# bharath-raghavan/enflow

Measured on AMD Instinct MI355X. Metric: molecule-transforms/sec (fwd+log|detJ|), batch 1024×22 atoms, 1/2/4/8 GPU, higher is better.
Workload: dtype f32 (f16x3 GEMMs); 1 GPU; lf_forward_1024x22_L8_H128_nf5_f32; molecules_per_gpu=1024, atoms_per_molecule=22, coupling_layers=8, hidden_nf=128, node_nf=5, global_batch=1024, parallelism=single GPU

## Files before the change

enflow_amd/_lib.py:

```python
import ctypes
import os

import torch

_HERE = os.path.dirname(os.path.abspath(__file__))
LIB_PATH = os.environ.get("ENFLOW_LIB") or os.path.join(_HERE, "libenflow_hip.so")
LIB_NF16_PATH = os.environ.get("ENFLOW_LIB_NF16") or os.path.join(_HERE, "libenflow_hip_nf16.so")
BASE_NFMAX = 8
MAX_NODE_NF = 16
TRAIN_MAX_NODE_NF = 16

ERR_TOO_MANY_ATOMS = 1
ERR_FEW_IMAGES = 2
ERR_TOO_MANY_FEATURES = 4
ERR_RANGE = 8
ERR_SMALL = 16
ERR_HANDOFF = 32
ERR_RERUN = ERR_RANGE | ERR_SMALL
DEQUANT_NONE, DEQUANT_ARGMAX, DEQUANT_FLOOR = 0, 1, 2
PREC_F32, PREC_F16X3, PREC_BF16 = 0, 1, 2
PRECISIONS = {"f32": PREC_F32, "f16x3": PREC_F16X3, "bf16": PREC_BF16}
PREC_NO_SPLIT = 0x400
EGCL_ATTENTION, EGCL_NORM_DIFF, EGCL_TANH, EGCL_ACT = 1, 2, 4, 8
EGCL_VARIANTS = 0x100
BWD_F32 = 0x200

_i, _i64, _f, _p = ctypes.c_int, ctypes.c_int64, ctypes.c_float, ctypes.c_void_p
_u64 = ctypes.c_uint64

SIGNATURES = {
    "enflow_abi_version": (_i, []),
    "enflow_set_latency_threshold": (_i, [_i]),
    "enflow_latency_threshold": (_i, []),
    "enflow_set_split_threshold": (_i, [_i]),
    "enflow_set_fs_threshold": (_i, [_i]),
    "enflow_set_handoff_spin_limit": (_i, [_i]),
    "enflow_set_dequant_ahead": (_i, [_i]),
    "enflow_set_longest_first": (_i, [_i]),
    "enflow_longest_first_order_f32": (_i, [_i, _i, _p, _p, _p, _p, _i, _i, _p, _p, _p]),
    "enflow_max_atoms": (_i, []),
    "enflow_max_node_nf": (_i, []),
    "enflow_supports_hidden": (_i, [_i]),
    "enflow_egcl_packed_size": (_i64, [_i, _i]),
    "enflow_argmax_packed_size": (_i64, [_i, _i]),
    "enflow_pack_egcl_f32": (_i, [_p, _i, _i, _p, _p]),
    "enflow_pack_egcl_ex_f32": (_i, [_p, _i, _i, _i, _p, _p, _p]),
    "enflow_pack_egcl_act_f32": (_i, [_p, _i, _i, _i, _i, _f, _f, _p, _p, _p]),
    "enflow_pack_argmax_f32": (_i, [_p, _i, _i, _p, _p]),
    "enflow_lf_forward_f32": (_i, [_i, _i, _i, _i, _i, _p, _p, _p, _p, _p, _p, _p, _p, _i,
                                   _i, _p, _p, _f, _f, _f, _p, _p, _p, _p, _p, _p, _i, _p]),
    "enflow_lf_reverse_f32": (_i, [_i, _i, _i, _i, _i, _p, _p, _p, _p, _p, _p, _p, _p, _i,
                                   _i, _f, _f, _p, _p, _p, _i, _p]),
    "enflow_lf_forward_io_f32": (_i, [_i, _i, _i, _i, _i, _p, _p, _p, _p, _p, _p, _p, _p, _p, _p, _p, _p, _i,
                                      _i, _p, _p, _u64, _u64, _f, _f, _f, _p, _p, _p, _p, _p, _p, _p, _i, _p]),
    "enflow_lf_reverse_io_f32": (_i, [_i, _i, _i, _i, _i, _p, _p, _p, _p, _p, _p, _p, _p, _p, _p, _p, _p, _i,
                                      _i, _f, _f, _p, _p, _p, _i, _p]),
    "enflow_lf_forward_io2_f32": (_i, [_i, _i, _i, _i, _i, _p, _p, _p, _p, _p, _p, _p, _p, _p, _p, _p, _p, _i,
                                       _i, _p, _p, _u64, _u64, _f, _f, _f, _p, _p, _p, _p, _p, _p, _p, _i,
                                       _p, _p, _i, _p]),
    "enflow_lf_reverse_io2_f32": (_i, [_i, _i, _i, _i, _i, _p, _p, _p, _p, _p, _p, _p, _p, _p, _p, _p, _p, _i,
                                       _i, _f, _f, _p, _p, _p, _i, _p, _p, _i, _p]),
    "enflow_lf_large_workspace_size": (_i64, [_i, _i, _i, _i]),
    "enflow_lf_forward_large_f32": (_i, [_i, _i, _i, _i, _i, _p, _p, _p, _p, _p, _p, _p, _p, _i,
                                         _i, _p, _p, _f, _f, _f, _p, _p, _p, _i, _p, _p, _p, _i64, _p]),
    "enflow_lf_reverse_large_f32": (_i, [_i, _i, _i, _i, _i, _p, _p, _p, _p, _p, _p, _p, _p, _i,
                                         _i, _f, _f, _p, _p, _p, _i, _p, _i64, _p]),
    "enflow_egcl_forward_large_f32": (_i, [_i, _i, _i, _i, _i, _p, _p, _p, _p, _p, _p, _f,
                                           _p, _p, _p, _p, _i, _p, _i64, _p]),
    "enflow_neighbour_pairs_large_f32": (_i, [_i, _i, _i, _p, _p, _p, _p, _p, _p, _p, _p, _i64, _p]),
    "enflow_edge_list_workspace_size": (_i64, [_i, _i]),
    "enflow_edge_list_count_f32": (_i, [_i, _i, _p, _p, _p, _p, _p, _p, _p, _i64, _p]),
# ... 55 lines not shown
        return LIB_PATH
    if int(nf) <= MAX_NODE_NF:
        return LIB_NF16_PATH
    raise NotImplementedError(f"enflow_amd kernels are built for node_nf <= {MAX_NODE_NF} (got {nf})")


def lib(nf=None):
    path = lib_path(nf)
    handle = _libs.get(path)
    if handle is None:
        if not os.path.exists(path):
            raise HipPathError(
                f"{path} is missing: build it with "
                "`python -c 'import __graft_entry__ as g; g.build()'` (hipcc --offload-arch=gfx950)")
        handle = ctypes.CDLL(path)
        for name, (res, args) in SIGNATURES.items():
            if not hasattr(handle, name):
                continue
            fn = getattr(handle, name)
            fn.restype = res
            fn.argtypes = args
        if _lat_threshold[0] is not None and hasattr(handle, "enflow_set_latency_threshold"):
            handle.enflow_set_latency_threshold(_lat_threshold[0])
        if _split_threshold[0] is not None and hasattr(handle, "enflow_set_split_threshold"):
            handle.enflow_set_split_threshold(_split_threshold[0])
        if _fs_threshold[0] is not None and hasattr(handle, "enflow_set_fs_threshold"):
            handle.enflow_set_fs_threshold(_fs_threshold[0])
        if _spin_limit[0] is not None and hasattr(handle, "enflow_set_handoff_spin_limit"):
            handle.enflow_set_handoff_spin_limit(_spin_limit[0])
        if _dq_ahead[0] is not None and hasattr(handle, "enflow_set_dequant_ahead"):
            handle.enflow_set_dequant_ahead(_dq_ahead[0])
        if _longest_first[0] is not None and hasattr(handle, "enflow_set_longest_first"):
            handle.enflow_set_longest_first(_longest_first[0])
        _libs[path] = handle
    return handle


_lat_threshold = [None]


def set_latency_threshold(max_mols):
    prev = _lat_threshold[0]
    _lat_threshold[0] = int(max_mols)
    for h in _libs.values():
        if hasattr(h, "enflow_set_latency_threshold"):
            h.enflow_set_latency_threshold(int(max_mols))
    return prev


_split_threshold = [None]
_fs_threshold = [None]
_spin_limit = [None]
_dq_ahead = [None]


def set_dequant_ahead(on):
    prev = _dq_ahead[0]
    _dq_ahead[0] = 1 if on else 0
    for h in _libs.values():
        if hasattr(h, "enflow_set_dequant_ahead"):
            h.enflow_set_dequant_ahead(_dq_ahead[0])
    return prev


_longest_first = [None]


def set_longest_first(mode):
    prev = _longest_first[0]
    _longest_first[0] = int(mode)
    for h in _libs.values():
        if hasattr(h, "enflow_set_longest_first"):
            h.enflow_set_longest_first(int(mode))
    return prev


def longest_first_order(mol_ptr, r_cut, box, pos, max_mol_atoms, reverse=False, training=False):
    num_mols = int(mol_ptr.numel()) - 1
    keys = torch.full((max(num_mols, 1),), -1, dtype=torch.int32, device=pos.device)
    order = torch.full((max(num_mols, 1),), -1, dtype=torch.int32, device=pos.device)
    rc = lib().enflow_longest_first_order_f32(num_mols, int(max_mol_atoms), ptr(mol_ptr), ptr(r_cut), ptr(box),
                                              ptr(pos), int(bool(reverse)), int(bool(training)), ptr(keys),
                                              ptr(order), stream_ptr(pos.device))
    if rc < 0:
        raise HipPathError(f"enflow_longest_first_order_f32 failed with code {rc}")
    return keys[:num_mols], order[:num_mols], bool(rc)


def set_handoff_spin_limit(polls):
    prev = _spin_limit[0]
    _spin_limit[0] = int(polls)
    for h in _libs.values():
        if hasattr(h, "enflow_set_handoff_spin_limit"):
            h.enflow_set_handoff_spin_limit(int(polls))
    return prev


def set_split_threshold(max_mols):
    prev = _split_threshold[0]
    _split_threshold[0] = int(max_mols)
    for h in _libs.values():
        if hasattr(h, "enflow_set_split_threshold"):
            h.enflow_set_split_threshold(int(max_mols))
    return prev


# ... 186 lines not shown
```

enflow_amd/csrc/enflow_flow.hip:

```cpp

#include <mutex>
#include "enflow_large.h"
#include "enflow_host.h"
#include "enflow_latency.h"
#include "enflow_split.h"

__device__ __forceinline__ void pack_egcl_body(const float* __restrict__ raw, int H, int nf, float* __restrict__ out,
                                               int flags, const float* __restrict__ att, int act_kind, float act_p0,
                                               float act_p1) {
  const EgclLayout L = egcl_layout(H, nf);
  const RawEgcl R = raw_egcl(H, nf);
  const int NT = H / 32;
  const int K1 = 2 * nf + 1;
  for (int idx = blockIdx.x * blockDim.x + threadIdx.x; idx < L.total; idx += gridDim.x * blockDim.x) {
    float v = 0.f;
    if (idx < L.we2f) {
      int e = idx - L.we1f;
      int lane = e & 63, slot = (e >> 6) % (NFMAX + 1), t = (e >> 6) / (NFMAX + 1);
      int hh = lane >> 5;
      int q = -1;
      if (slot < NFMAX / 2) { int f = 2 * slot + hh; if (f < nf) q = f; }
      else if (slot < NFMAX) { int f = 2 * (slot - NFMAX / 2) + hh; if (f < nf) q = nf + f; }
      else if (hh == 0) q = 2 * nf;
      if (q >= 0) v = raw[R.We1 + (32 * t + (lane & 31)) * K1 + q];
// ... 544 lines not shown
    *b = DqBuf{dev, st, 0, 0, nullptr, nullptr};
  }
  if (b->cap_z < nz) {
    float* p = nullptr;
    const size_t c = nz < 65536 ? 65536 : nz;
    if (hipMalloc(&p, c * sizeof(float)) != hipSuccess) return nullptr;
    b->z = p;
    b->cap_z = c;
  }
  if (b->cap_m < nm) {
    float* p = nullptr;
    const size_t c = nm < 4096 ? 4096 : nm;
    if (hipMalloc(&p, c * sizeof(float)) != hipSuccess) return nullptr;
    b->lq = p;
    b->cap_m = c;
  }
  return b;
}
static int g_cus[64];
static int cus_now() {
  int dev = 0;
  if (hipGetDevice(&dev) != hipSuccess) return 0;
  if (dev < 0 || dev >= 64) return 0;
  if (g_cus[dev] == 0) {
    int cus = 0;
    if (hipDeviceGetAttribute(&cus, hipDeviceAttributeMultiprocessorCount, dev) != hipSuccess || cus <= 0) return 0;
    g_cus[dev] = cus;
  }
  return g_cus[dev];
}
static int lat_threshold_now() { return g_lat_threshold >= 0 ? g_lat_threshold : cus_now(); }

static int g_longest_first = LONGEST_FIRST_DEFAULT;
struct OrdBuf {
  int dev;
  hipStream_t st;
  size_t cap;
  int32_t* key;
};
static OrdBuf g_ord[64];
static int g_nord = 0;
static int32_t* order_buffers(hipStream_t st, size_t nm) {
  int dev = 0;
  if (hipGetDevice(&dev) != hipSuccess) return nullptr;
  std::lock_guard<std::mutex> lk(g_dq_mu);
  OrdBuf* b = nullptr;
  for (int i = 0; i < g_nord; ++i)
    if (g_ord[i].dev == dev && g_ord[i].st == st) b = &g_ord[i];
  if (!b) {
    if (g_nord >= 64) return nullptr;
    b = &g_ord[g_nord++];
    *b = OrdBuf{dev, st, 0, nullptr};
  }
  if (b->cap < nm) {
    int32_t* p = nullptr;
    const size_t c = nm < 4096 ? 4096 : nm;
    if (hipMalloc(&p, 2 * c * sizeof(int32_t)) != hipSuccess) return nullptr;
    b->key = p;
    b->cap = c;
  }
  return b->key;
}
static bool longest_first_applies(int NN, int grid, bool rev, bool tape) {
  if (g_longest_first == 0 || NN > 64 || grid < 1 || grid > ORDER_MAX_MOLS) return false;
  if (g_longest_first >= 2) return true;
  (void)rev;
  return NN == 32 && !tape && grid > 2 * cus_now();
}
template <int NN>
static void launch_order(int num_mols, hipStream_t st, const FlowArgs& A, int32_t* keys, int32_t* order) {
  ENFLOW_TIMED("order_key_kernel", st,
               hipLaunchKernelGGL((order_key_kernel<NN>), dim3(num_mols), dim3(BLOCK), 0, st, A, keys));
  ENFLOW_TIMED("order_rank_kernel", st,
               hipLaunchKernelGGL(order_rank_kernel, dim3((num_mols + 63) / 64), dim3(BLOCK), 0, st, keys, num_mols,
                                  order));
}

template <int HH, int NN, int RBB, bool REV>
static void launch_flow(int prec, int num_mols, hipStream_t st, const FlowArgs& A0) {
  if (NN == 32 && !(prec & ENFLOW_PREC_NO_SPLIT) && enflow_fs_launch(HH, REV, prec, num_mols, st, &A0)) return;
  prec &= ~ENFLOW_PREC_NO_SPLIT;
  FlowArgs A = A0;
  if constexpr (RBB == NN && NN <= 64) {
    if (A.mol_list == nullptr && longest_first_applies(NN, num_mols, REV, A.tape != nullptr)) {
      int32_t* const buf = order_buffers(st, (size_t)A.num_mols);
      if (buf != nullptr && A.num_mols == num_mols) {
        launch_order<NN>(num_mols, st, A, buf, buf + num_mols);
        A.order = buf + num_mols;
      }
    }
  }
  if (NN == 32 && num_mols <= lat_threshold_now() && enflow_lat_launch(HH, REV, prec, num_mols, st, &A)) return;
  if (prec & ENFLOW_EGCL_VARIANTS) launch_flow_v<HH, NN, RBB, REV, true>(prec & 0xff, num_mols, st, A);
  else launch_flow_v<HH, NN, RBB, REV, false>(prec, num_mols, st, A);
}

extern "C" {

#ifdef ENFLOW_STAMPS
int enflow_read_stamps(unsigned long long* host_out, int reset) {
  if (hipMemcpyFromSymbol(host_out, HIP_SYMBOL(enflow_stamp_acc), sizeof(unsigned long long) * NSTAMP) != hipSuccess)
    return -2;
  if (reset) {
    unsigned long long z[NSTAMP] = {0};
    if (hipMemcpyToSymbol(HIP_SYMBOL(enflow_stamp_acc), z, sizeof(z)) != hipSuccess) return -2;
  }
  return NSTAMP;
}
#endif

#ifdef ENFLOW_STAMPS
int enflow_read_dq_stamps(unsigned long long* host_out, int reset) {
  if (hipMemcpyFromSymbol(host_out, HIP_SYMBOL(enflow_dq_stamp_acc), sizeof(unsigned long long) * 8) != hipSuccess)
    return -2;
  if (reset) {
    unsigned long long z[8] = {0};
    if (hipMemcpyToSymbol(HIP_SYMBOL(enflow_dq_stamp_acc), z, sizeof(z)) != hipSuccess) return -2;
  }
  return 8;
}
#endif

int enflow_abi_version(void) { return ENFLOW_ABI; }
int enflow_set_dequant_ahead(int on) {
  const int prev = g_dq_ahead;
  g_dq_ahead = on ? 1 : 0;
  return prev;
}
int enflow_set_longest_first(int mode) {
  const int prev = g_longest_first;
  g_longest_first = mode < 0 ? 0 : (mode > 2 ? 2 : mode);
  return prev;
}
int enflow_longest_first_order_f32(int num_mols, int max_mol_atoms, const int32_t* mol_ptr, const float* r_cut,
                                   const float* box, const float* pos, int reverse, int training,
                                   int32_t* keys, int32_t* order, void* stream) {
  if (num_mols < 0 || max_mol_atoms < 0 || (num_mols > 0 && (!mol_ptr || !r_cut || !box || !pos || !keys || !order)))
    return -1;
  if (max_mol_atoms > 64 || num_mols > ORDER_MAX_MOLS) return 0;
  const int NN = max_mol_atoms <= 32 ? 32 : 64;
  const int applies = longest_first_applies(NN, num_mols, reverse != 0, training != 0) ? 1 : 0;
  if (num_mols == 0) return applies;
  FlowArgs A{mol_ptr, r_cut, box, nullptr, nullptr, const_cast<float*>(pos), nullptr, nullptr, 0, 1,
             0, nullptr, nullptr, 0.f, 0.f, 0.f, nullptr, nullptr, nullptr, nullptr, nullptr};
  A.num_mols = num_mols;
  if (NN == 32) launch_order<32>(num_mols, S(stream), A, keys, order);
  else launch_order<64>(num_mols, S(stream), A, keys, order);
  return hipGetLastError() == hipSuccess ? applies : -2;
}
int enflow_set_latency_threshold(int max_mols) {
  const int prev = g_lat_threshold;
  g_lat_threshold = max_mols < 0 ? -1 : max_mols;
  return prev;
}
int enflow_latency_threshold(void) { return lat_threshold_now(); }
int enflow_max_atoms(void) { return MAX_ATOMS; }
int enflow_max_node_nf(void) { return NFMAX; }
int enflow_supports_hidden(int hidden_nf) { return hid_ok(hidden_nf); }

int64_t enflow_egcl_packed_size(int hidden_nf, int node_nf) {
  if (!hid_ok(hidden_nf) || node_nf < 1 || node_nf > NFMAX) return -1;
  return egcl_layout(hidden_nf, node_nf).total;
}
int64_t enflow_argmax_packed_size(int hidden_nf, int node_nf) {
// ... 306 lines not shown
```

enflow_amd/csrc/flow_device.h:

```cpp
#pragma once

#include <hip/hip_runtime.h>
#include <stdint.h>
#include <math.h>
#include <type_traits>

#include "enflow_hip.h"
#include "enflow_timing.h"

#define ENFLOW_ABI 13
#ifndef WAVES
#define WAVES 4
#endif
#define BLOCK (64 * WAVES)
#ifndef ENFLOW_NFMAX
#define ENFLOW_NFMAX 8
#endif
#define NFMAX ENFLOW_NFMAX
static_assert(NFMAX == 8 || NFMAX == 16, "ENFLOW_NFMAX must be 8 or 16");
#define KS0MAX (NFMAX / 8 + 1)
#ifndef ENFLOW_MSG_MFMA
#define ENFLOW_MSG_MFMA 1
#endif
#define NFP (NFMAX + 1)
#ifndef ENFLOW_WAVES_PER_SIMD
#define ENFLOW_WAVES_PER_SIMD 2
#endif

typedef float f32x16 __attribute__((ext_vector_type(16)));
typedef float f32x4 __attribute__((ext_vector_type(4)));

__host__ __device__ constexpr int rho(int r, int hh) { return (r & 3) + 8 * (r >> 2) + 4 * hh; }

__host__ __device__ inline int node_ksteps(int H, int nf) { return (H + nf + 1) / 2; }

struct EgclLayout {
  int we1f, we2f, wc1f, wn1h, wn1a, wv1f, wn2f, be1, be2, bc1, wc2, bn1, bv1, wv2, bn2, bv2, watt, batt, vfl,
      scl, we1x, wv1x, wn1hx, wn1ax, wn2x, we2x, wc1x, we2b, wc1b, total;
};

enum { EGCL_ATTENTION = 1, EGCL_NORM_DIFF = 2, EGCL_TANH = 4 };

enum { PREC_F32 = 0, PREC_F16X3 = 1, PREC_BF16 = 2 };

__host__ __device__ inline EgclLayout egcl_layout(int H, int nf) {
  (void)nf;
  const int NT = H / 32;
  EgclLayout L;
  int o = 0;
  L.we1f = o; o += NT * (NFMAX + 1) * 64;
  L.we2f = o; o += H * H;
  L.wc1f = o; o += H * H;
  L.wn1h = o; o += NT * (NFMAX / 2) * 64;
  L.wn1a = o; o += NT * (H / 8) * 256;
  L.wv1f = o; o += NT * (NFMAX / 2) * 64;
// ... 796 lines not shown
#pragma unroll
    for (int g4 = 0; g4 < 4; ++g4) {
      const f32x4 v = ld4(b + 32 * t + 8 * g4 + 4 * hh);
#pragma unroll
      for (int u = 0; u < 4; ++u) acc[t][4 * g4 + u] = v[u];
    }
}

template <int NT>
__device__ __forceinline__ void bias_silu(f32x16 (&X)[NT], const float* __restrict__ bias, int hh) {
#pragma unroll
  for (int t = 0; t < NT; ++t)
#pragma unroll
    for (int g4 = 0; g4 < 4; ++g4) {
      const f32x4 b = *reinterpret_cast<const f32x4*>(bias + 32 * t + 8 * g4 + 4 * hh);
#pragma unroll
      for (int u = 0; u < 4; ++u) X[t][4 * g4 + u] = silu_f(X[t][4 * g4 + u] + b[u]);
      __builtin_amdgcn_sched_barrier(0);
    }
}

#if defined(ENFLOW_STAMPS) || (defined(ENFLOW_STAMPS_BWD) && defined(ENFLOW_BACKWARD_TU))
#define NSTAMP 20
__device__ unsigned long long enflow_stamp_acc[NSTAMP];
#define STAMP_DECL unsigned long long st_prev = __builtin_amdgcn_s_memtime(), st_acc[NSTAMP] = {0};
#define STAMP_ARGS , unsigned long long& st_prev, unsigned long long (&st_acc)[NSTAMP]
#define STAMP_PASS , st_prev, st_acc
#define STAMP(k)                                               \
  do {                                                         \
    unsigned long long now_ = __builtin_amdgcn_s_memtime();    \
    st_acc[k] += now_ - st_prev;                               \
    st_prev = now_;                                            \
  } while (0)
#define STAMP_FLUSH                                                              \
  if (threadIdx.x == 0)                                                          \
    for (int k_ = 0; k_ < NSTAMP; ++k_) atomicAdd(&enflow_stamp_acc[k_], st_acc[k_]);
#else
#define STAMP_DECL
#define STAMP_ARGS
#define STAMP_PASS
#define STAMP(k) do {} while (0)
#define STAMP_FLUSH
#endif

template <int H, int NMAX, int RB = NMAX, bool BWD = false>
struct Smem {
  static constexpr int NT = H / 32;
  static constexpr int AST = BWD ? H + 3 : H + 4;
  static constexpr bool BLOCKED = RB < NMAX;
  static constexpr bool PACKC = BLOCKED || BWD;
  static constexpr int MAXP = RB * (NMAX - 1);
  static constexpr int PC = BLOCKED ? 512 : MAXP;
  static constexpr int CW = PACKC ? (RB * NMAX + 1) / 2 : RB * NMAX;
  static constexpr int NETA = BWD ? 1 : (BLOCKED ? RB : NMAX);
  static constexpr int NBCH = 8;
  static constexpr int NBW = BWD ? (NBCH * 2 * H > WAVES * NMAX * (NFMAX + 3) ? NBCH * 2 * H
                                                                             : WAVES * NMAX * (NFMAX + 3))
                                 : 1;
  float pos[NMAX * 3], vel[NMAX * 3], boxa[BLOCKED ? 3 : NMAX * 3];
  float h[NMAX * NFP], g[NMAX * NFP], G[BWD ? 1 : NMAX * NFP];
  float Q[NMAX];
  float F[BLOCKED ? NMAX * 3 : 1];
  alignas(16) float bias[4 * H];
  static constexpr bool W1X_LDS = !BLOCKED && !BWD && NMAX <= 32;
  alignas(16) float w1x[W1X_LDS ? NT * KS0MAX * 512 : 4];
  alignas(16) float agg[RB * AST];
  alignas(16) float head[BWD ? 1 : WAVES][BWD ? 1 : H + 4];
  uint32_t pairs[PC];
  uint32_t mask27[NMAX];
  static constexpr bool IMG_LDS = W1X_LDS && NT * KS0MAX * 512 >= NMAX * 27 * 4;
  uint32_t near27[IMG_LDS ? NMAX : 1];
  float bbox[8];
  int idmap[NMAX];
  int cntrow[NMAX];
  int headrow[WAVES];
  int ishead[WAVES];
  int scan[WAVES];
  int npairs;
  int ptotal;
  int err;
  uint32_t big;
  float red[WAVES];
  static constexpr int NDT = BWD ? 1 : NT, NDR = BWD ? 1 : RB;
  static constexpr bool MSG_MMA = ENFLOW_MSG_MFMA && !BWD && NMAX == 32 && RB == 32;
  static constexpr int MIS = 34;
  union {
    int C[CW];
    struct {
      alignas(16) uint32_t img[MSG_MMA ? WAVES : 1][MSG_MMA ? 32 * MIS : 1];
      alignas(16) uint32_t tb[MSG_MMA ? WAVES : 1][32];
      int rt[MSG_MMA ? WAVES : 1][32];
    } mm;
    struct { float qp[NDT][NDR]; float gp[NDT][NFMAX][NDR]; } nd;
    float net[NETA * 2 * NFMAX];
    float nb[NBW];
  } u;
};

template <class S>
__device__ __forceinline__ int c_get(const S& sm, int e) {
  if constexpr (S::PACKC) return (sm.u.C[e >> 1] >> (16 * (e & 1))) & 0xffff;
  else return sm.u.C[e];
}
template <class S>
__device__ __forceinline__ void c_add(S& sm, int e, int v) {
  if constexpr (S::PACKC) atomicAdd(&sm.u.C[e >> 1], v << (16 * (e & 1)));
  else atomicAdd(&sm.u.C[e], v);
}

struct MolRef {
  int a0, n;
  float rc;
  float bx, by, bz;
  int m = 0;
};

__device__ __forceinline__ float shift_of(int idx, float b) { return idx == 0 ? -b : (idx == 1 ? b : 0.f); }

template <class S>
__device__ __forceinline__ void build_images(S& sm, const MolRef& M, int tid) {
  const int n = M.n;
  const float rx = M.bx + M.rc, ry = M.by + M.rc, rz = M.bz + M.rc;
  for (int a = tid; a < n; a += BLOCK) {
    sm.mask27[a] = 0u;
// ... 164 lines not shown
    }
  }
  if (tid == BLOCK - 1) {
    int tot = 0;
    for (int k = 0; k < WAVES; ++k) tot += sm.scan[k];
    sm.ptotal = tot;
    sm.npairs = min(tot - p0, PC);
  }
  __syncthreads();
  return sm.ptotal;
}

template <class S>
__device__ __forceinline__ void build_block_pairs(S& sm, const MolRef& M, int tid, int r0, int rb) {
  static_assert(!S::BLOCKED, "blocked images compact in passes (block_compact)");
  block_counts(sm, M, tid, r0, rb, r0 == 0 && rb == M.n);
  block_compact(sm, M.n, tid, rb, 0);
}

template <class S>
__device__ __forceinline__ void build_pairs(S& sm, const MolRef& M, int tid) {
  static_assert(!S::BLOCKED, "build_pairs needs the unblocked image");
  build_images(sm, M, tid);
  build_block_pairs(sm, M, tid, 0, M.n);
}

template <bool BIG>
__device__ __forceinline__ int pair_row(uint32_t pr) { return BIG ? (int)(pr & 31u) : (int)(pr & 0xffu); }

template <int H, int NMAX, int RB, int PREC = PREC_F32, bool VAR = false, bool BIG = false, class Pre = NoMid>
__device__ __forceinline__ void edge_tiles(Smem<H, NMAX, RB>& sm, const float* __restrict__ Lp, const EgclLayout& L,
                                           const MolRef& M, int nf, int tid, int r0, int rb,
                                           bool zero_agg STAMP_ARGS, const float* __restrict__ cpos = nullptr,
                                           const float* __restrict__ ch = nullptr, Pre&& pre = NoMid{}) {
  constexpr int NT = H / 32;
  constexpr int AST = Smem<H, NMAX, RB>::AST;
  const int lane = tid & 63, w = __builtin_amdgcn_readfirstlane(tid >> 6);
  const int j = lane & 31, hh = lane >> 5;
  const int P = sm.npairs;
  const int T = (P + 31) >> 5;
  const int tpw = (T + WAVES - 1) / WAVES;

  if (zero_agg)
    for (int e = tid; e < rb * AST; e += BLOCK) sm.agg[e] = 0.f;
  for (int e = tid; e < WAVES * (H + 4); e += BLOCK) (&sm.head[0][0])[e] = 0.f;
  const float K0 = PREC != PREC_F32 ? Lp[L.scl + 4] : 1.f;
  const float K1 = PREC == PREC_F16X3 ? Lp[L.scl + 0] : 1.f;
  const float K2 = PREC == PREC_F16X3 ? Lp[L.scl + 2] : 1.f;
  for (int k = tid; k < H; k += BLOCK) {
    sm.bias[k] = Lp[L.be1 + k] * K0;
    sm.bias[H + k] = Lp[L.be2 + k] * K1;
    sm.bias[2 * H + k] = Lp[L.bc1 + k] * K2;
    sm.bias[3 * H + k] = Lp[L.wc2 + k];
  }
  if constexpr (PREC != PREC_F32 && Smem<H, NMAX, RB>::W1X_LDS) {
    const int ks_n = gemm0_ksteps(nf);
    for (int e = tid; e < NT * ks_n * 128; e += BLOCK) {
      const int blk = e >> 7, r = e & 127, ln = r >> 1, part = r & 1;
      const int t = blk / ks_n, ks = blk - t * ks_n;
      const f32x4 v = ld4(Lp + L.we1x + (t * KS0MAX + ks) * 512 + ln * 8 + part * 4);
      st4(&sm.w1x[(t * KS0MAX + ks) * 512 + part * 256 + ln * 4], v);
    }
  }
  if (tid < WAVES) {
    const int t0 = tid * tpw;
    int hr = -1, ih = 0;
    if (t0 < T) {
      const int p0 = t0 * 32;
      hr = pair_row<BIG>(sm.pairs[p0]);
      ih = (p0 > 0) && (pair_row<BIG>(sm.pairs[p0 - 1]) == hr);
    }
    sm.headrow[tid] = hr;
    sm.ishead[tid] = ih;
  }
  __syncthreads();

  const int t0 = w * tpw, t1 = min(T, t0 + tpw);
  const int headrow = sm.headrow[w];
  const bool ishead = sm.ishead[w] != 0;
  const int nh = (nf + 1) >> 1;
  const rsrc_t W = weights_rsrc(Lp, L.total);
  const float hbx = M.bx * 0.5f, hby = M.by * 0.5f, hbz = M.bz * 0.5f;
  constexpr float NLOG2E = -1.4426950408889634f;
  const float ik0 = PREC != PREC_F32 ? Lp[L.scl + 5] : 1.f;
  const float ik1 = PREC == PREC_F16X3 ? Lp[L.scl + 1] : 1.f;
  const float ik2 = PREC == PREC_F16X3 ? Lp[L.scl + 3] : 1.f;
  const float c0 = NLOG2E * ik0, c1 = NLOG2E * ik1, c2 = NLOG2E * ik2;
  constexpr bool MMA = PREC != PREC_F32 && !VAR && !BIG && Smem<H, NMAX, RB>::MSG_MMA;
  constexpr int XD = (NMAX == 32 && RB == 32 && WAVES == 4 && !BIG) ? ENFLOW_FWD_X3_DEPTH : ENFLOW_X3_DEPTH;
  constexpr int MIS = Smem<H, NMAX, RB>::MIS;
  const int vfl = VAR ? (int)Lp[L.vfl] : 0;
  const bool v_att = (vfl & EGCL_ATTENTION) != 0, v_nd = (vfl & EGCL_NORM_DIFF) != 0,
             v_tanh = (vfl & EGCL_TANH) != 0;
  const Act act = VAR ? act_of(Lp + L.vfl + 1) : act_silu();

  bool range_bad = false;
  constexpr bool GUARD = PREC == PREC_F16X3;
  uint32_t bigw = 0u;
  STAMP(8);
  for (int tile = t0; tile < t1; ++tile) {
    const int p = tile * 32 + j;
    const bool valid = p < P;
    uint32_t o0 = 0u, o1 = 0u, o2 = 0u;
    const uint32_t vmask = valid ? ENFLOW_BIG_BITS : 0u;
    auto seen_big = [&](uint32_t o, uint32_t kind) {
      if constexpr (GUARD) bigw |= __ballot((o & vmask) != 0u) ? kind : 0u;
    };
    const uint32_t pr = valid ? sm.pairs[p] : 0u;
    const int il = pair_row<BIG>(pr);
    const int jl = BIG ? (int)((pr >> 5) & 0x3fffffu) : (int)((pr >> 8) & 0xffu);
// ... 288 lines not shown
                                             e[t + 1][4 * g4 + 3]}, c1, K1, ik1, act);
#pragma unroll
          for (int u = 0; u < 4; ++u) e[t + 1][4 * g4 + u] = y[u];
        }
      }, NoMid{}, [&](int, const f16x8& bh, const f16x8&) {
        if constexpr (GUARD) o2 = or_hi(o2, bh);
      });
      seen_big(o2, BIGK_M);
#pragma unroll
      for (int tp = 0; tp < NT; ++tp)
#pragma unroll
        for (int g4 = 0; g4 < 4; ++g4) {
          const f32x4 w2 = *reinterpret_cast<const f32x4*>(sm.bias + 3 * H + 32 * tp + 8 * g4 + 4 * hh);
          const f32x4 y = act4s<VAR>((f32x4){hc[tp][4 * g4], hc[tp][4 * g4 + 1], hc[tp][4 * g4 + 2],
                                             hc[tp][4 * g4 + 3]}, c2, K2, ik2, act);
#pragma unroll
          for (int u = 0; u < 4; ++u) part += w2[u] * y[u];
        }
    }
    float phi = part + __shfl_xor(part, 32, 64);
    if constexpr (PREC != PREC_F32) range_bad |= valid && !__builtin_isfinite(phi);
    if (v_tanh) phi = tanhf(phi);
    const float nd = v_nd ? __builtin_amdgcn_rcpf(sqrtf(radial) + 1.f) : 1.f;
    f32x4* const fslot = reinterpret_cast<f32x4*>(dst_row + H);
    const f32x4 fold = *fslot;
    float tx = c * clamp100(dx * nd * phi);
    float ty = c * clamp100(dy * nd * phi);
    float tz = c * clamp100(dz * nd * phi);
    float tw = 0.f;
    seg_scan4x(tx, ty, tz, tw, SE);
    if (seg_end && hh == 0) *fslot = fold + (f32x4){tx, ty, tz, tw};
    STAMP(14);
  }
  if constexpr (PREC != PREC_F32) {
    if (__ballot(range_bad))
      if (lane == 0) atomicOr(&sm.err, ENFLOW_ERR_RANGE);
  }
  if constexpr (GUARD) {
    if (lane == 0 && t1 > t0) atomicOr(&sm.big, bigw | (uint32_t)BIGK_EDGE);
  }
  pre();
  __syncthreads();
  STAMP(15);
  for (int f = tid; f < H + 3; f += BLOCK) {
    for (int ww = 0; ww < WAVES; ++ww)
      if (sm.ishead[ww]) sm.agg[sm.headrow[ww] * AST + f] += sm.head[ww][f];
  }
  __syncthreads();
}

template <int H, int NMAX, int RB>
__device__ __forceinline__ void node_partials_reduce(Smem<H, NMAX, RB>& sm, const float* __restrict__ Lp,
                                                     const EgclLayout& L, int nf, int tid, int r0, int rb) {
  constexpr int NT = H / 32;
  const float bv2 = Lp[L.bv2];
  for (int a = tid; a < rb; a += BLOCK) {
    float s = 0.f;
#pragma unroll
    for (int tp = 0; tp < NT; ++tp) s += sm.u.nd.qp[tp][a];
    sm.Q[r0 + a] = s + bv2;
  }
  for (int e = tid; e < rb * nf; e += BLOCK) {
    const int a = e / nf, q = e - a * nf;
    float s = 0.f;
#pragma unroll
    for (int tp = 0; tp < NT; ++tp) s += sm.u.nd.gp[tp][q][a];
    sm.G[(r0 + a) * NFP + q] = s + Lp[L.bn2 + q];
  }
  __syncthreads();
}

template <int H, int NMAX, int RB, bool VAR = false>
// ... 425 lines not shown
  float* h;
  float* g;
  float* pos;
  float* vel;
  const float* layers;
  int n_layers;
  int nf;
  int dequant_kind;
  const float* dequant;
  const float* noise;
  float dequant_scale;
  float dt;
  float cw;
  float* ldj_mol;
  int32_t* argmax_idx;
  int32_t* max_idx;
  int32_t* err;
  unsigned long long* stats;
  float* tape;
  int32_t* pair_counts;
  int num_mols, num_atoms;
  const float* h_in = nullptr;
  const float* g_in = nullptr;
  const float* pos_in = nullptr;
  const float* vel_in = nullptr;
  unsigned long long seed = 0, offset = 0;
  uint32_t* ticket = nullptr;
  float* ldj_total = nullptr;
  double ldj_cst = 0.0;
  int32_t* mol_err = nullptr;
  const int32_t* mol_list = nullptr;
  const float* lq_mol = nullptr;
  const int32_t* order = nullptr;
  __device__ __forceinline__ NoiseSrc noise_src() const { return NoiseSrc{noise, seed, offset}; }
};

enum { LOAD_POS = 1, LOAD_H = 2, LOAD_VELG = 4 };

template <int H, int NMAX, int RB>
__device__ __forceinline__ bool load_molecule(Smem<H, NMAX, RB>& sm, const FlowArgs& A, MolRef& M, int what) {
  const int32_t* const map = A.mol_list ? A.mol_list : A.order;
  const int m = map ? map[blockIdx.x] : (int)blockIdx.x;
  const int tid = threadIdx.x;
  M.m = m;
  M.a0 = A.mol_ptr[m];
  M.n = A.mol_ptr[m + 1] - M.a0;
  M.rc = 0.f;
  M.bx = M.by = M.bz = 0.f;
  if (M.n > NMAX || A.nf > NFMAX) {
    if (tid == 0) {
      const int e = M.n > NMAX ? ENFLOW_ERR_TOO_MANY_ATOMS : ENFLOW_ERR_TOO_MANY_FEATURES;
      atomicOr(A.err, e);
      if (A.mol_err) atomicOr(&A.mol_err[m], e);
    }
    return false;
  }
  const int n = M.n, nf = A.nf;
  if (what & LOAD_POS) {
    M.rc = A.r_cut[m];
    for (int e = tid; e < n * 3; e += BLOCK) {
      sm.pos[e] = (A.pos_in ? A.pos_in : A.pos)[(size_t)M.a0 * 3 + e];
      if (!Smem<H, NMAX, RB>::BLOCKED || e < 3) sm.boxa[e] = A.box[(size_t)M.a0 * 3 + e];
    }
  }
  if (what & LOAD_VELG)
    for (int e = tid; e < n * 3; e += BLOCK) sm.vel[e] = (A.vel_in ? A.vel_in : A.vel)[(size_t)M.a0 * 3 + e];
// ... 22 lines not shown
```

enflow_amd/csrc/flow_kernel.h:

```cpp
#pragma once

#ifndef ENFLOW_BLOCKED_WPS
#define ENFLOW_BLOCKED_WPS ENFLOW_WAVES_PER_SIMD
#endif
__device__ __forceinline__ void ticket_reduce_ldj(const FlowArgs& A, double* red, int* last) {
  const int tid = threadIdx.x;
  __threadfence();
  __syncthreads();
  if (tid == 0) *last = atomicAdd(A.ticket, 1u) == gridDim.x - 1;
  __syncthreads();
  if (!*last) return;
  __threadfence();
  constexpr int RT = 256;
  double s = 0.0;
  if (tid < RT)
    for (int m = tid; m < A.num_mols; m += RT) s += (double)__builtin_nontemporal_load(&A.ldj_mol[m]);
  if (tid < RT) red[tid] = s;
  __syncthreads();
  for (int off = RT / 2; off > 0; off >>= 1) {
    if (tid < off) red[tid] += red[tid + off];
    __syncthreads();
  }
  if (tid == 0) {
    A.ldj_total[0] = (float)(red[0] + A.ldj_cst);
// ... 53 lines not shown
        for (int d = 0; d < 3; ++d)
          sm.pos[a * 3 + d] = pbc1(sm.pos[a * 3 + d] - sm.vel[a * 3 + d] * A.dt, pbox(a, d));
      }
      __syncthreads();
    }
    build_images(sm, Ml, tid_l);
    STAMP(3);
    int npairs_layer = 0;
    auto block_pass = [&](const int r0, const int rb) {
      int tot;
      if constexpr (BLOCKED) {
        block_counts(sm, Ml, tid_l, r0, rb);
        tot = block_compact(sm, n, tid_l, rb, 0);
      } else {
        build_block_pairs(sm, Ml, tid_l, r0, rb);
        tot = sm.npairs;
      }
      STAMP(2);
      npairs_layer += tot;
      if (A.stats != nullptr && tid == 0) {
        unsigned long long edges = 0;
        for (int a = 0; a < rb; ++a) edges += (unsigned long long)sm.cntrow[r0 + a];
        atomicAdd(&A.stats[0], (unsigned long long)tot);
        atomicAdd(&A.stats[1], edges);
      }
      NodeFrags<H> nfr;
      constexpr bool EARLY = !BLOCKED && PREC != PREC_F32;
      const int wv = __builtin_amdgcn_readfirstlane(tid_l >> 6);
      auto pre = [&] {
        if constexpr (EARLY) {
          if (wv < (H / 32) * (RB / 32)) nfr.issue(weights_rsrc(Lp, L.total), L, tid_l & 63, wv);
        }
      };
      edge_tiles<H, NMAX, RB, PREC, VAR>(sm, Lp, L, Ml, nf, tid_l, r0, rb, true STAMP_PASS, nullptr, nullptr, pre);
      if constexpr (BLOCKED) {
        constexpr int PC = Smem<H, NMAX, RB>::PC;
        for (int p0 = PC; p0 < tot; p0 += PC) {
          block_compact(sm, n, tid_l, rb, p0);
          edge_tiles<H, NMAX, RB, PREC, VAR>(sm, Lp, L, Ml, nf, tid_l, r0, rb, false STAMP_PASS);
        }
      }
      STAMP(4);
      {
        if constexpr (PREC != PREC_F32)
          node_phase_x3_f<H, NMAX, RB, VAR>(sm, Lp, L, n, nf, tid_l, r0, rb, nfr, EARLY);
        else node_phase<H, NMAX, RB, VAR>(sm, Lp, L, n, nf, tid_l, r0, rb);
      }
      STAMP(5);
      if constexpr (PREC == PREC_F16X3) {
        if (tid == 0) {
          if (small_operands(sm.big)) sm.err |= ENFLOW_ERR_SMALL;
          sm.big = 0u;
        }
      }
      if (!REV && A.tape != nullptr) {
        const TapeLayout T = tape_layout(A.num_atoms, nf, H, A.n_layers);
        const size_t la = (size_t)l * A.num_atoms + M.a0 + r0;
        float* hx = A.tape + T.hx + la * T.ldhx;
        for (int e = tid; e < rb * T.ldhx; e += BLOCK) {
          const int a = e / T.ldhx, c = e - a * T.ldhx;
          hx[e] = c < nf ? sm.h[(r0 + a) * NFP + c] : sm.agg[a * AST + (c - nf)];
        }
        for (int e = tid; e < rb * nf; e += BLOCK) {
          const int a = e / nf, q = e - a * nf;
          A.tape[T.g + la * nf + e] = sm.g[(r0 + a) * NFP + q];
        }
        for (int e = tid; e < rb * 3; e += BLOCK) {
// ... 114 lines not shown
```

include/enflow_hip.h:

```cpp
#ifndef ENFLOW_HIP_H
#define ENFLOW_HIP_H

#include <stdint.h>

#ifdef __cplusplus
extern "C" {
#endif

#define ENFLOW_ERR_TOO_MANY_ATOMS   1
#define ENFLOW_ERR_FEW_IMAGES       2
#define ENFLOW_ERR_TOO_MANY_FEATURES 4
#define ENFLOW_ERR_RANGE            8
#define ENFLOW_ERR_SMALL           16
#define ENFLOW_ERR_HANDOFF         32

#define ENFLOW_PREC_F32   0
#define ENFLOW_PREC_F16X3 1
#define ENFLOW_PREC_BF16  2
#define ENFLOW_PREC_NO_SPLIT 0x400

#define ENFLOW_DEQUANT_NONE   0
#define ENFLOW_DEQUANT_ARGMAX 1
#define ENFLOW_DEQUANT_FLOOR  2

int enflow_abi_version(void);

int enflow_set_latency_threshold(int max_mols);
int enflow_latency_threshold(void);

int enflow_set_split_threshold(int max_mols);
int enflow_set_fs_threshold(int max_mols);
int enflow_set_handoff_spin_limit(int polls);
int enflow_set_dequant_ahead(int on);
int enflow_set_longest_first(int mode);
int enflow_longest_first_order_f32(int num_mols, int max_mol_atoms, const int32_t* mol_ptr, const float* r_cut,
                                   const float* box, const float* pos, int reverse, int training,
                                   int32_t* keys, int32_t* order, void* stream);

int enflow_max_atoms(void);
int enflow_max_node_nf(void);
int enflow_supports_hidden(int hidden_nf);

int64_t enflow_egcl_packed_size(int hidden_nf, int node_nf);
int64_t enflow_argmax_packed_size(int hidden_nf, int node_nf);

int enflow_pack_egcl_f32(const float* raw, int hidden_nf, int node_nf,
                         float* packed, void* stream);

#define ENFLOW_EGCL_ATTENTION 1
#define ENFLOW_EGCL_NORM_DIFF 2
#define ENFLOW_EGCL_TANH      4
#define ENFLOW_EGCL_ACT       8
#define ENFLOW_EGCL_VARIANTS 0x100

int enflow_pack_egcl_ex_f32(const float* raw, int hidden_nf, int node_nf, int flags,
                            const float* att, float* packed, void* stream);

#define ENFLOW_ACT_SILU        0
#define ENFLOW_ACT_RELU        1
#define ENFLOW_ACT_LEAKY_RELU  2
#define ENFLOW_ACT_ELU         3
#define ENFLOW_ACT_CELU        4
#define ENFLOW_ACT_SELU        5
#define ENFLOW_ACT_GELU        6
#define ENFLOW_ACT_GELU_TANH   7
#define ENFLOW_ACT_TANH        8
#define ENFLOW_ACT_SIGMOID     9
// ... 227 lines not shown
```

Baseline: 1.409 million molecule-transforms/s.

## Process leftover edge tiles cooperatively across all four waves

```diff
diff --git a/enflow_amd/_lib.py b/enflow_amd/_lib.py
--- a/enflow_amd/_lib.py
+++ b/enflow_amd/_lib.py
@@ -37,6 +37,7 @@
     "enflow_set_handoff_spin_limit": (_i, [_i]),
     "enflow_set_dequant_ahead": (_i, [_i]),
     "enflow_set_longest_first": (_i, [_i]),
+    "enflow_set_coop_tiles": (_i, [_i]),
     "enflow_longest_first_order_f32": (_i, [_i, _i, _p, _p, _p, _p, _i, _i, _p, _p, _p]),
     "enflow_max_atoms": (_i, []),
     "enflow_max_node_nf": (_i, []),
@@ -158,6 +159,8 @@
             handle.enflow_set_dequant_ahead(_dq_ahead[0])
         if _longest_first[0] is not None and hasattr(handle, "enflow_set_longest_first"):
             handle.enflow_set_longest_first(_longest_first[0])
+        if _coop_tiles[0] is not None and hasattr(handle, "enflow_set_coop_tiles"):
+            handle.enflow_set_coop_tiles(_coop_tiles[0])
         _libs[path] = handle
     return handle
 
@@ -198,6 +201,18 @@
     for h in _libs.values():
         if hasattr(h, "enflow_set_longest_first"):
             h.enflow_set_longest_first(int(mode))
+    return prev
+
+
+_coop_tiles = [None]
+
+
+def set_coop_tiles(on):
+    prev = _coop_tiles[0]
+    _coop_tiles[0] = 1 if on else 0
+    for h in _libs.values():
+        if hasattr(h, "enflow_set_coop_tiles"):
+            h.enflow_set_coop_tiles(_coop_tiles[0])
     return prev
 
 
diff --git a/enflow_amd/csrc/enflow_flow.hip b/enflow_amd/csrc/enflow_flow.hip
--- a/enflow_amd/csrc/enflow_flow.hip
+++ b/enflow_amd/csrc/enflow_flow.hip
@@ -600,6 +600,7 @@
 static int lat_threshold_now() { return g_lat_threshold >= 0 ? g_lat_threshold : cus_now(); }
 
 static int g_longest_first = LONGEST_FIRST_DEFAULT;
+static int g_coop_tiles = 1;
 struct OrdBuf {
   int dev;
   hipStream_t st;
@@ -649,6 +650,7 @@
   if (NN == 32 && !(prec & ENFLOW_PREC_NO_SPLIT) && enflow_fs_launch(HH, REV, prec, num_mols, st, &A0)) return;
   prec &= ~ENFLOW_PREC_NO_SPLIT;
   FlowArgs A = A0;
+  A.coop_tiles = g_coop_tiles;
   if constexpr (RBB == NN && NN <= 64) {
     if (A.mol_list == nullptr && longest_first_applies(NN, num_mols, REV, A.tape != nullptr)) {
       int32_t* const buf = order_buffers(st, (size_t)A.num_mols);
@@ -698,6 +700,11 @@
 int enflow_set_longest_first(int mode) {
   const int prev = g_longest_first;
   g_longest_first = mode < 0 ? 0 : (mode > 2 ? 2 : mode);
+  return prev;
+}
+int enflow_set_coop_tiles(int on) {
+  const int prev = g_coop_tiles;
+  g_coop_tiles = on ? 1 : 0;
   return prev;
 }
 int enflow_longest_first_order_f32(int num_mols, int max_mol_atoms, const int32_t* mol_ptr, const float* r_cut,
diff --git a/enflow_amd/csrc/flow_device.h b/enflow_amd/csrc/flow_device.h
--- a/enflow_amd/csrc/flow_device.h
+++ b/enflow_amd/csrc/flow_device.h
@@ -21,6 +21,9 @@
 #define KS0MAX (NFMAX / 8 + 1)
 #ifndef ENFLOW_MSG_MFMA
 #define ENFLOW_MSG_MFMA 1
+#endif
+#ifndef COOP_RC
+#define COOP_RC 2
 #endif
 #define NFP (NFMAX + 1)
 #ifndef ENFLOW_WAVES_PER_SIMD
@@ -883,14 +886,16 @@
     st_acc[k] += now_ - st_prev;                               \
     st_prev = now_;                                            \
   } while (0)
+#define STAMP_ADD(k, v) do { st_acc[k] += (unsigned long long)(v); } while (0)
 #define STAMP_FLUSH                                                              \
-  if (threadIdx.x == 0)                                                          \
+  if (threadIdx.x == 0)                                                       \
     for (int k_ = 0; k_ < NSTAMP; ++k_) atomicAdd(&enflow_stamp_acc[k_], st_acc[k_]);
 #else
 #define STAMP_DECL
 #define STAMP_ARGS
 #define STAMP_PASS
 #define STAMP(k) do {} while (0)
+#define STAMP_ADD(k, v) do {} while (0)
 #define STAMP_FLUSH
 #endif
 
@@ -935,12 +940,14 @@
   static constexpr int NDT = BWD ? 1 : NT, NDR = BWD ? 1 : RB;
   static constexpr bool MSG_MMA = ENFLOW_MSG_MFMA && !BWD && NMAX == 32 && RB == 32;
   static constexpr int MIS = 34;
+  static constexpr bool COOP_LDS = MSG_MMA && WAVES == 4 && H == 128;
   union {
     int C[CW];
     struct {
       alignas(16) uint32_t img[MSG_MMA ? WAVES : 1][MSG_MMA ? 32 * MIS : 1];
       alignas(16) uint32_t tb[MSG_MMA ? WAVES : 1][32];
       int rt[MSG_MMA ? WAVES : 1][32];
+      alignas(16) uint32_t xb[COOP_LDS ? 8 * 2 * 64 * 4 : 4];
     } mm;
     struct { float qp[NDT][NDR]; float gp[NDT][NFMAX][NDR]; } nd;
     float net[NETA * 2 * NFMAX];
@@ -1171,14 +1178,19 @@
 __device__ __forceinline__ void edge_tiles(Smem<H, NMAX, RB>& sm, const float* __restrict__ Lp, const EgclLayout& L,
                                            const MolRef& M, int nf, int tid, int r0, int rb,
                                            bool zero_agg STAMP_ARGS, const float* __restrict__ cpos = nullptr,
-                                           const float* __restrict__ ch = nullptr, Pre&& pre = NoMid{}) {
+                                           const float* __restrict__ ch = nullptr, Pre&& pre = NoMid{},
+                                           bool coop = false) {
   constexpr int NT = H / 32;
   constexpr int AST = Smem<H, NMAX, RB>::AST;
   const int lane = tid & 63, w = __builtin_amdgcn_readfirstlane(tid >> 6);
   const int j = lane & 31, hh = lane >> 5;
   const int P = sm.npairs;
   const int T = (P + 31) >> 5;
-  const int tpw = (T + WAVES - 1) / WAVES;
+  constexpr bool COOP = Smem<H, NMAX, RB>::COOP_LDS && PREC == PREC_F16X3 && !VAR && !BIG && NMAX == 32 &&
+                        RB == 32 && ENFLOW_MSG_MFMA;
+  const bool co = COOP && coop && (T & 3) != 0 && (T & 3) <= COOP_RC;
+  const int Tc = co ? (T & ~3) : T;
+  const int tpw = co ? (T >> 2) : (T + WAVES - 1) / WAVES;
 
   if (zero_agg)
     for (int e = tid; e < rb * AST; e += BLOCK) sm.agg[e] = 0.f;
@@ -1204,7 +1216,7 @@
   if (tid < WAVES) {
     const int t0 = tid * tpw;
     int hr = -1, ih = 0;
-    if (t0 < T) {
+    if (t0 < Tc) {
       const int p0 = t0 * 32;
       hr = pair_row<BIG>(sm.pairs[p0]);
       ih = (p0 > 0) && (pair_row<BIG>(sm.pairs[p0 - 1]) == hr);
@@ -1214,7 +1226,7 @@
   }
   __syncthreads();
 
-  const int t0 = w * tpw, t1 = min(T, t0 + tpw);
+  const int t0 = w * tpw, t1 = min(Tc, t0 + tpw);
   const int headrow = sm.headrow[w];
   const bool ishead = sm.ishead[w] != 0;
   const int nh = (nf + 1) >> 1;
@@ -1569,12 +1581,230 @@
     if (seg_end && hh == 0) *fslot = fold + (f32x4){tx, ty, tz, tw};
     STAMP(14);
   }
+  STAMP_ADD(18, t1 - t0);
+  if constexpr (COOP) {
+    if (co) {
+      auto& mm = sm.u.mm;
+      uint32_t* const xa = &mm.xb[0];
+      const int vo = lane * 32;
+      uint32_t* const img = &mm.img[w][0];
+      const int ibase = (8 * hh + ((lane >> 2) & 3)) * MIS + 2 * (4 * ((lane >> 4) & 1) + (lane & 3));
+      auto frag_off = [&](int off_floats, int ts) {
+        return (off_floats + ((w * NT + (ts >> 1)) * 2 + (ts & 1)) * 512) * 4;
+      };
+      for (int tile = Tc; tile < T; ++tile) {
+        if (tile > Tc) __syncthreads();
+        const int p = tile * 32 + j;
+        const bool valid = p < P;
+        uint32_t o0 = 0u, o1 = 0u, o2 = 0u;
+        const uint32_t vmask = valid ? ENFLOW_BIG_BITS : 0u;
+        auto seen_big = [&](uint32_t o, uint32_t kind) { bigw |= __ballot((o & vmask) != 0u) ? kind : 0u; };
+        const uint32_t pr = valid ? sm.pairs[p] : 0u;
+        const int il = (int)(pr & 0xffu), jl = (int)((pr >> 8) & 0xffu);
+        const int i = r0 + il;
+        const float c = (float)(pr >> 16);
+        const int row = valid ? il : -1 - j;
+        const SegExec SE = seg_exec(row);
+        const int row_prev = __shfl_up(row, 1, 32);
+        const bool start = j == 0 || row_prev != row;
+        const uint32_t S = (uint32_t)__ballot(start);
+        const int seg = __builtin_popcount(S & (uint32_t)((2ull << j) - 1ull)) - 1;
+        const int nseg = __builtin_popcount(S);
+        if (hh == 0) {
+          mm.tb[w][j] = ((uint32_t)__builtin_bit_cast(uint16_t, (_Float16)c) << 16) | (uint32_t)seg;
+          if (start) mm.rt[w][seg] = valid ? il : -1;
+        }
+        const int row_next = __shfl_down(row, 1, 32);
+        const bool seg_end = valid && (j == 31 || row_next != row);
+        float* const dst_row = &sm.agg[(valid ? il : 0) * AST];
+        const float dx = pbc1(sm.pos[i * 3 + 0] - sm.pos[jl * 3 + 0], hbx);
+        const float dy = pbc1(sm.pos[i * 3 + 1] - sm.pos[jl * 3 + 1], hby);
+        const float dz = pbc1(sm.pos[i * 3 + 2] - sm.pos[jl * 3 + 2], hbz);
+        const float radial = dx * dx + dy * dy + dz * dz;
+        f32x4 fh[2 * NT], fl[2 * NT];
+#pragma unroll
+        for (int ts = 0; ts < 2 * NT; ++ts) {
+          fh[ts] = bload4(W, vo, frag_off(L.we2x, ts));
+          fl[ts] = bload4(W, vo + 16, frag_off(L.we2x, ts));
+        }
+        f32x16 x0;
+#pragma unroll
+        for (int g4 = 0; g4 < 4; ++g4) {
+          const f32x4 v = ld4(sm.bias + 32 * w + 8 * g4 + 4 * hh);
+#pragma unroll
+          for (int u = 0; u < 4; ++u) x0[4 * g4 + u] = v[u];
+        }
+        const int ks_n = gemm0_ksteps(nf), nch = gemm0_nch(nf);
+        for (int ks = 0; ks < ks_n; ++ks) {
+          f32x16 in;
+          if (ks < nch) {
+            const float* hrow = &sm.h[(hh ? jl : i) * NFP + 8 * ks];
+#pragma unroll
+            for (int jj = 0; jj < 8; ++jj) in[jj] = hrow[jj];
+            if (hh && ks == nch - 1 && gemm0_radial_slot7(nf)) in[7] = radial;
+          } else {
+#pragma unroll
+            for (int jj = 0; jj < 8; ++jj) in[jj] = 0.f;
+            if (hh == 0) in[0] = radial;
+          }
+          f16x8 bh, bl;
+          split_f16(in, 0, bh, bl);
+          o0 = or_hi(o0, bh);
+          const f32x4 ah = ld4(&sm.w1x[(w * KS0MAX + ks) * 512 + lane * 4]);
+          const f32x4 al = ld4(&sm.w1x[(w * KS0MAX + ks) * 512 + 256 + lane * 4]);
+          x0 = mfma_f16(ah, bh, x0);
+          x0 = mfma_f16(ah, bl, x0);
+          x0 = mfma_f16(al, bh, x0);
+        }
+        seen_big(o0, BIGK_X0);
+        auto publish = [&](f32x16& X, float cc, float KK, float ikk, bool image) {
+#pragma unroll
+          for (int g4 = 0; g4 < 4; ++g4) {
+            const f32x4 y = act4s<VAR>((f32x4){X[4 * g4], X[4 * g4 + 1], X[4 * g4 + 2], X[4 * g4 + 3]}, cc, KK,
+                                       ikk, act);
+#pragma unroll
+            for (int u = 0; u < 4; ++u) X[4 * g4 + u] = y[u];
+          }
+#pragma unroll
+          for (int s = 0; s < 2; ++s) {
+            f16x8 bh, bl;
+            split_f16(X, s, bh, bl);
+            const u32x4v hv = __builtin_bit_cast(u32x4v, bh), lv = __builtin_bit_cast(u32x4v, bl);
+            if (image) {
+              uint32_t* const r = img + j * MIS + 2 * hh + 8 * s;
+              *reinterpret_cast<u32x2v*>(r) = (u32x2v){hv[0], hv[1]};
+              *reinterpret_cast<u32x2v*>(r + 4) = (u32x2v){hv[2], hv[3]};
+              *reinterpret_cast<u32x2v*>(r + 16) = (u32x2v){lv[0], lv[1]};
+              *reinterpret_cast<u32x2v*>(r + 20) = (u32x2v){lv[2], lv[3]};
+            } else {
+              *reinterpret_cast<u32x4v*>(xa + (((2 * w + s) * 2 + 0) * 64 + lane) * 4) = hv;
+              *reinterpret_cast<u32x4v*>(xa + (((2 * w + s) * 2 + 1) * 64 + lane) * 4) = lv;
+            }
+          }
+        };
+        auto chain = [&](f32x16& acc, const float* bias, bool image, uint32_t& o) {
+#pragma unroll
+          for (int g4 = 0; g4 < 4; ++g4) {
+            const f32x4 v = ld4(bias + 32 * w + 8 * g4 + 4 * hh);
+#pragma unroll
+            for (int u = 0; u < 4; ++u) acc[4 * g4 + u] = v[u];
+          }
+#pragma unroll
+          for (int ts = 0; ts < 2 * NT; ++ts) {
+            u32x4v hv, lv;
+            if (image) {
+              const uint32_t* const r = &mm.img[ts >> 1][0] + j * MIS + 2 * hh + 8 * (ts & 1);
+              const u32x2v h0 = *reinterpret_cast<const u32x2v*>(r), h1 = *reinterpret_cast<const u32x2v*>(r + 4);
+              const u32x2v l0 = *reinterpret_cast<const u32x2v*>(r + 16), l1 = *reinterpret_cast<const u32x2v*>(r + 20);
+              hv = (u32x4v){h0[0], h0[1], h1[0], h1[1]};
+              lv = (u32x4v){l0[0], l0[1], l1[0], l1[1]};
+            } else {
+              hv = *reinterpret_cast<const u32x4v*>(xa + ((ts * 2 + 0) * 64 + lane) * 4);
+              lv = *reinterpret_cast<const u32x4v*>(xa + ((ts * 2 + 1) * 64 + lane) * 4);
+            }
+            const f16x8 bh = __builtin_bit_cast(f16x8, hv), bl = __builtin_bit_cast(f16x8, lv);
+            o = or_hi(o, bh);
+            acc = mfma_f16(fh[ts], bh, acc);
+            acc = mfma_f16(fh[ts], bl, acc);
+            acc = mfma_f16(fl[ts], bh, acc);
+          }
+        };
+        publish(x0, c0, K0, ik0, false);
+        __syncthreads();
+        f32x16 e;
+        chain(e, sm.bias + H, false, o1);
+        seen_big(o1, BIGK_Y0);
+#pragma unroll
+        for (int ts = 0; ts < 2 * NT; ++ts) {
+          fh[ts] = bload4(W, vo, frag_off(L.wc1x, ts));
+          fl[ts] = bload4(W, vo + 16, frag_off(L.wc1x, ts));
+        }
+        publish(e, c1, K1, ik1, true);
+        __syncthreads();
+        u32x4v tq[4];
+        const uint32_t* const tb = &mm.tb[w][0];
+#pragma unroll
+        for (int q = 0; q < 4; ++q) tq[q] = *reinterpret_cast<const u32x4v*>(tb + 16 * (q >> 1) + 8 * hh + 4 * (q & 1));
+        const int rn = mm.rt[w][j];
+        f16x8 sel[2];
+#pragma unroll
+        for (int ks = 0; ks < 2; ++ks) {
+          const u32x4v q0 = tq[2 * ks], q1 = tq[2 * ks + 1];
+          const uint32_t wv[8] = {q0[0], q0[1], q0[2], q0[3], q1[0], q1[1], q1[2], q1[3]};
+          u32x4v pk;
+#pragma unroll
+          for (int i2 = 0; i2 < 4; ++i2) {
+            const uint32_t a0 = (wv[2 * i2] & 0xffffu) == (uint32_t)j ? wv[2 * i2] >> 16 : 0u;
+            const uint32_t a1 = (wv[2 * i2 + 1] & 0xffffu) == (uint32_t)j ? wv[2 * i2 + 1] & 0xffff0000u : 0u;
+            pk[i2] = a0 | a1;
+          }
+          sel[ks] = __builtin_bit_cast(f16x8, pk);
+        }
+        const bool vn = j < nseg && rn >= 0;
+        float* dstn = &sm.agg[0];
+        if (vn) dstn = &sm.agg[rn * AST];
+        s16x4 ar[4][2];
+#pragma unroll
+        for (int k = 0; k < 4; ++k)
+#pragma unroll
+          for (int rd = 0; rd < 2; ++rd) ar[k][rd] = lds_tr16(img + ibase + (16 * (k >> 1) + 4 * rd) * MIS + 16 * (k & 1));
+        f32x16 Y;
+#pragma unroll
+        for (int g4 = 0; g4 < 4; ++g4) {
+          const f32x4 v = ld4(dstn + 32 * w + 8 * g4 + 4 * hh);
+#pragma unroll
+          for (int u = 0; u < 4; ++u) Y[4 * g4 + u] = v[u];
+        }
+#pragma unroll
+        for (int k = 0; k < 4; ++k)
+          Y = __builtin_amdgcn_mfma_f32_32x32x16_f16(cat_f16x8(ar[k][0], ar[k][1]), sel[k >> 1], Y, 0, 0, 0);
+        f32x16 hc;
+        chain(hc, sm.bias + 2 * H, true, o2);
+        seen_big(o2, BIGK_M);
+        if (vn) {
+#pragma unroll
+          for (int g4 = 0; g4 < 4; ++g4)
+            st4(dstn + 32 * w + 8 * g4 + 4 * hh, (f32x4){Y[4 * g4], Y[4 * g4 + 1], Y[4 * g4 + 2], Y[4 * g4 + 3]});
+        }
+        float* const yb = reinterpret_cast<float*>(xa);
+#pragma unroll
+        for (int g4 = 0; g4 < 4; ++g4)
+          st4(yb + ((w * 4 + g4) * 64 + lane) * 4,
+              act4s<VAR>((f32x4){hc[4 * g4], hc[4 * g4 + 1], hc[4 * g4 + 2], hc[4 * g4 + 3]}, c2, K2, ik2, act));
+        __syncthreads();
+        if (w == 0) {
+          float part = 0.f;
+#pragma unroll
+          for (int tp = 0; tp < NT; ++tp)
+#pragma unroll
+            for (int g4 = 0; g4 < 4; ++g4) {
+              const f32x4 w2 = *reinterpret_cast<const f32x4*>(sm.bias + 3 * H + 32 * tp + 8 * g4 + 4 * hh);
+              const f32x4 y = ld4(yb + ((tp * 4 + g4) * 64 + lane) * 4);
+#pragma unroll
+              for (int u = 0; u < 4; ++u) part += w2[u] * y[u];
+            }
+          const float phi = part + __shfl_xor(part, 32, 64);
+          range_bad |= valid && !__builtin_isfinite(phi);
+          f32x4* const fslot = reinterpret_cast<f32x4*>(dst_row + H);
+          const f32x4 fold = *fslot;
+          float tx = c * clamp100(dx * phi);
+          float ty = c * clamp100(dy * phi);
+          float tz = c * clamp100(dz * phi);
+          float tw = 0.f;
+          seg_scan4x(tx, ty, tz, tw, SE);
+          if (seg_end && hh == 0) *fslot = fold + (f32x4){tx, ty, tz, tw};
+        }
+      }
+      STAMP_ADD(17, T - Tc);
+      STAMP(16);
+    }
+  }
   if constexpr (PREC != PREC_F32) {
     if (__ballot(range_bad))
       if (lane == 0) atomicOr(&sm.err, ENFLOW_ERR_RANGE);
   }
   if constexpr (GUARD) {
-    if (lane == 0 && t1 > t0) atomicOr(&sm.big, bigw | (uint32_t)BIGK_EDGE);
+    if (lane == 0 && (t1 > t0 || co)) atomicOr(&sm.big, bigw | (uint32_t)BIGK_EDGE);
   }
   pre();
   __syncthreads();
@@ -2066,6 +2296,7 @@
   const int32_t* mol_list = nullptr;
   const float* lq_mol = nullptr;
   const int32_t* order = nullptr;
+  int coop_tiles = 0;
   __device__ __forceinline__ NoiseSrc noise_src() const { return NoiseSrc{noise, seed, offset}; }
 };
 
diff --git a/enflow_amd/csrc/flow_kernel.h b/enflow_amd/csrc/flow_kernel.h
--- a/enflow_amd/csrc/flow_kernel.h
+++ b/enflow_amd/csrc/flow_kernel.h
@@ -109,7 +109,9 @@
           if (wv < (H / 32) * (RB / 32)) nfr.issue(weights_rsrc(Lp, L.total), L, tid_l & 63, wv);
         }
       };
-      edge_tiles<H, NMAX, RB, PREC, VAR>(sm, Lp, L, Ml, nf, tid_l, r0, rb, true STAMP_PASS, nullptr, nullptr, pre);
+      const bool coop = A.coop_tiles != 0 && (REV || A.tape == nullptr);
+      edge_tiles<H, NMAX, RB, PREC, VAR>(sm, Lp, L, Ml, nf, tid_l, r0, rb, true STAMP_PASS, nullptr, nullptr, pre,
+                                         coop);
       if constexpr (BLOCKED) {
         constexpr int PC = Smem<H, NMAX, RB>::PC;
         for (int p0 = PC; p0 < tot; p0 += PC) {
diff --git a/include/enflow_hip.h b/include/enflow_hip.h
--- a/include/enflow_hip.h
+++ b/include/enflow_hip.h
@@ -33,6 +33,7 @@
 int enflow_set_handoff_spin_limit(int polls);
 int enflow_set_dequant_ahead(int on);
 int enflow_set_longest_first(int mode);
+int enflow_set_coop_tiles(int on);
 int enflow_longest_first_order_f32(int num_mols, int max_mol_atoms, const int32_t* mol_ptr, const float* r_cut,
                                    const float* box, const float* pos, int reverse, int training,
                                    int32_t* keys, int32_t* order, void* stream);
```

Result: faster. 1.445 million molecule-transforms/s (median of 6 runs) (+2.6%).
